# modin-project/modin

Hardware: AMD Instinct MI355X
Metric: rows/sec groupby-sum (higher is better)
Workload: dtype f64; 1 GPU; groupby-sum-1e9-int64key-f64val; rows=1000000000, key_cardinality=1000000, key_distribution=uniform, key_dtype=int64, val_dtype=float64, partitions_per_rank=1, api_layer=modin_amd.pandas DataFrame.groupby('k').sum(), parallelism=dp1

## Files before the change

include/hipframe.h:

```cpp
#ifndef HIPFRAME_H
#define HIPFRAME_H

#include <stdint.h>
#include <stddef.h>

#ifdef __cplusplus
extern "C" {
#endif

enum {
  HF_OK = 0,
  HF_ERR_HIP = 1,
  HF_ERR_ARG = 2,
  HF_ERR_NOINIT = 3,
  HF_ERR_UNSUPPORTED = 4
};

enum {
  HF_INT64 = 0,
  HF_FLOAT64 = 1
};

typedef struct hf_col hf_col;

// ... 51 lines not shown
  double  mn, mx;
  int64_t isum, imn, imx;
} hf_reduce_result;
int hf_reduce(const hf_col* in, hf_reduce_result* out);

enum { HF_AGG_SUM = 0, HF_AGG_MIN = 1, HF_AGG_MAX = 2,
       HF_AGG_PROD = 3  };
int hf_groupby_accum(const hf_col* keys,
                     const hf_col* const* vals,
                     int nvals, int agg_op,
                     int64_t key_min, int64_t n_slots,
                     uintptr_t sums, uintptr_t rowcnt, uintptr_t counts);

int hf_group_moments(const hf_col* gid,
                     const hf_col* val,
                     uintptr_t centre, int64_t n_groups, uintptr_t table);

int hf_fill_f64(uintptr_t dptr, double value, int64_t n);
int hf_fill_i64(uintptr_t dptr, int64_t value, int64_t n);

int hf_fill_randint(hf_col* col, uint64_t seed, int64_t lo, int64_t hi);
int hf_fill_randf64(hf_col* col, uint64_t seed);
int hf_fill_randcdf(hf_col* col, uint64_t seed, const hf_col* cdf);

int hf_groupby_hash_accum(const hf_col* keys, const hf_col* const* vals,
                          int nvals, int agg_op, int64_t H,
                          uintptr_t tkey, uintptr_t sums, uintptr_t rowcnt,
                          uintptr_t counts);
int hf_groupby_hash_compact(uintptr_t tkey, uintptr_t sums, uintptr_t rowcnt,
                            uintptr_t counts, int nvals, int64_t H,
                            hf_col** out_keys, hf_col** out_sums,
                            hf_col** out_counts, int64_t* n_groups);

int hf_groupby_sorted(const hf_col* sorted_keys, const hf_col* const* vals,
                      int nvals, int agg_op, int want_counts,
                      hf_col** out_keys, hf_col** out_sums,
                      hf_col** out_counts, int64_t* n_groups);

int hf_fixup_empty(const hf_col* val, const hf_col* cnt, hf_col** out);

int hf_groupby_compact(uintptr_t sums, uintptr_t rowcnt, uintptr_t counts,
                       int nvals, int64_t key_min, int64_t n_slots,
                       hf_col** out_keys,
                       hf_col** out_sums,
                       hf_col** out_counts,
                       int64_t* n_groups);

int hf_groupby_reduce(const hf_col* keys, const hf_col* const* vals,
                      int nvals, int agg_op, int want_counts,
                      int64_t key_min, int64_t n_slots,
                      hf_col** out_keys, hf_col** out_sums,
                      hf_col** out_counts, int64_t* n_groups);

typedef struct hf_join hf_join;

int hf_join_build(const hf_col* rkeys,
                  const hf_col* const* rvals,
                  int nr, int64_t key_min, int64_t n_slots, hf_join** out);
int hf_join_free(hf_join* j);

int hf_join_probe(const hf_join* j, const hf_col* lkeys,
                  hf_col** out_keys,
                  hf_col** out_lidx,
                  hf_col** out_rcols,
                  int64_t* n_out);

int hf_gather(const hf_col* col, const hf_col* idx, hf_col** out);

int hf_col_concat(const hf_col* const* cols, int ncols, hf_col** out);

int hf_col_slice(const hf_col* col, int64_t start, int64_t len, hf_col** out);

enum {
  HF_CMP_GT = 0, HF_CMP_GE = 1, HF_CMP_LT = 2, HF_CMP_LE = 3,
  HF_CMP_EQ = 4, HF_CMP_NE = 5,
  HF_CMP_NOTNA = 6
};
int hf_compare_scalar(int op, const hf_col* col, double scalar,
                      hf_col** out);

typedef struct hf_filterplan hf_filterplan;
int hf_filter_plan(const hf_col* mask, hf_filterplan** out, int64_t* n_kept);
int hf_filter_apply(const hf_filterplan* plan, const hf_col* col,
                    hf_col** out);
int hf_filter_iota(const hf_filterplan* plan, int64_t base, hf_col** out);
int hf_filter_plan_free(hf_filterplan* plan);

int hf_sort_perm(const hf_col* keys, int ascending, hf_col** out_perm);

int hf_shuffle_dest(const hf_col* keys, const int64_t* splitters, int nsplit,
                    hf_col** dest);

int hf_ordered_i64(const hf_col* col, int direction, hf_col** out);

int hf_cumsum(const hf_col* col, int agg_op, hf_col** out);

int hf_seg_cumsum(const hf_col* col, const hf_col* heads, int agg_op,
                  hf_col** out);

int hf_ewm_mean(const hf_col* col, const hf_col* heads ,
                double alpha, int adjust, int ignore_na, int64_t min_periods,
                hf_col** out);

int hf_scatter(const hf_col* col, const hf_col* idx, hf_col** out);

int hf_cross_idx(int64_t nl, int64_t nr, hf_col** lidx, hf_col** ridx);
// ... 15 lines not shown
```

modin_amd/core/lib.py:

```python

from __future__ import annotations

import ctypes as ct
import os
import threading

import numpy as np

_LIB_NAME = "libhipframe.so"


class HfError(RuntimeError):
    """Raised when a hipframe C-ABI call fails."""


class HfReduceResult(ct.Structure):
    _fields_ = [
        ("sum", ct.c_double),
        ("count", ct.c_int64),
        ("mn", ct.c_double),
        ("mx", ct.c_double),
        ("isum", ct.c_int64),
        ("imn", ct.c_int64),
        ("imx", ct.c_int64),
# ... 83 lines not shown
            "hf_groupby_hash_compact": (ct.c_int, [ct.c_size_t, ct.c_size_t,
                                                   ct.c_size_t, ct.c_size_t,
                                                   ct.c_int, ct.c_int64,
                                                   ct.POINTER(ct.c_void_p),
                                                   ct.POINTER(ct.c_void_p),
                                                   ct.POINTER(ct.c_void_p),
                                                   ct.POINTER(ct.c_int64)]),
            "hf_groupby_sorted": (ct.c_int, [ct.c_void_p,
                                             ct.POINTER(ct.c_void_p),
                                             ct.c_int, ct.c_int, ct.c_int,
                                             ct.POINTER(ct.c_void_p),
                                             ct.POINTER(ct.c_void_p),
                                             ct.POINTER(ct.c_void_p),
                                             ct.POINTER(ct.c_int64)]),
            "hf_search_sorted": (ct.c_int, [ct.c_void_p, ct.c_void_p,
                                            ct.POINTER(ct.c_void_p)]),
            "hf_ordered_i64": (ct.c_int, [ct.c_void_p, ct.c_int,
                                          ct.POINTER(ct.c_void_p)]),
            "hf_cumsum": (ct.c_int, [ct.c_void_p, ct.c_int,
                                     ct.POINTER(ct.c_void_p)]),
            "hf_seg_cumsum": (ct.c_int, [ct.c_void_p, ct.c_void_p, ct.c_int,
                                         ct.POINTER(ct.c_void_p)]),
            "hf_ewm_mean": (ct.c_int, [ct.c_void_p, ct.c_void_p, ct.c_double,
                                       ct.c_int, ct.c_int, ct.c_int64,
                                       ct.POINTER(ct.c_void_p)]),
            "hf_scatter": (ct.c_int, [ct.c_void_p, ct.c_void_p,
                                      ct.POINTER(ct.c_void_p)]),
            "hf_cross_idx": (ct.c_int, [ct.c_int64, ct.c_int64,
                                        ct.POINTER(ct.c_void_p),
                                        ct.POINTER(ct.c_void_p)]),
            "hf_shuffle_dest": (ct.c_int, [ct.c_void_p,
                                           ct.POINTER(ct.c_int64), ct.c_int,
                                           ct.POINTER(ct.c_void_p)]),
            "hf_memcpy_dd": (ct.c_int, [ct.c_size_t, ct.c_size_t,
                                        ct.c_int64]),
            "hf_sort_perm": (ct.c_int, [ct.c_void_p, ct.c_int,
                                        ct.POINTER(ct.c_void_p)]),
            "hf_fixup_empty": (ct.c_int, [ct.c_void_p, ct.c_void_p,
                                          ct.POINTER(ct.c_void_p)]),
            "hf_groupby_compact": (ct.c_int, [ct.c_size_t, ct.c_size_t, ct.c_size_t,
                                              ct.c_int, ct.c_int64, ct.c_int64,
                                              ct.POINTER(ct.c_void_p),
                                              ct.POINTER(ct.c_void_p),
                                              ct.POINTER(ct.c_void_p),
                                              ct.POINTER(ct.c_int64)]),
            "hf_groupby_reduce": (ct.c_int, [ct.c_void_p,
                                             ct.POINTER(ct.c_void_p),
                                             ct.c_int, ct.c_int, ct.c_int,
                                             ct.c_int64, ct.c_int64,
                                             ct.POINTER(ct.c_void_p),
                                             ct.POINTER(ct.c_void_p),
                                             ct.POINTER(ct.c_void_p),
                                             ct.POINTER(ct.c_int64)]),
            "hf_col_concat": (ct.c_int, [ct.POINTER(ct.c_void_p), ct.c_int,
                                         ct.POINTER(ct.c_void_p)]),
            "hf_col_slice": (ct.c_int, [ct.c_void_p, ct.c_int64, ct.c_int64,
                                        ct.POINTER(ct.c_void_p)]),
            "hf_join_build": (ct.c_int, [ct.c_void_p, ct.POINTER(ct.c_void_p),
                                         ct.c_int, ct.c_int64, ct.c_int64,
                                         ct.POINTER(ct.c_void_p)]),
            "hf_join_free": (ct.c_int, [ct.c_void_p]),
            "hf_join_probe": (ct.c_int, [ct.c_void_p, ct.c_void_p,
                                         ct.POINTER(ct.c_void_p),
                                         ct.POINTER(ct.c_void_p),
                                         ct.POINTER(ct.c_void_p),
                                         ct.POINTER(ct.c_int64)]),
            "hf_gather": (ct.c_int, [ct.c_void_p, ct.c_void_p,
                                     ct.POINTER(ct.c_void_p)]),
            "hf_compare_scalar": (ct.c_int, [ct.c_int, ct.c_void_p,
                                             ct.c_double,
                                             ct.POINTER(ct.c_void_p)]),
            "hf_filter_plan": (ct.c_int, [ct.c_void_p, ct.POINTER(ct.c_void_p),
                                          ct.POINTER(ct.c_int64)]),
            "hf_filter_apply": (ct.c_int, [ct.c_void_p, ct.c_void_p,
                                           ct.POINTER(ct.c_void_p)]),
            "hf_filter_iota": (ct.c_int, [ct.c_void_p, ct.c_int64,
                                          ct.POINTER(ct.c_void_p)]),
            "hf_filter_plan_free": (ct.c_int, [ct.c_void_p]),
            "hf_profiling": (ct.c_int, [ct.c_int]),
            "hf_kernel_stats": (ct.c_int, [ct.c_char_p, ct.POINTER(ct.c_int64),
                                           ct.POINTER(ct.c_double)]),
            "hf_kernel_stats_reset": (ct.c_int, []),
        }
        for name, (res, args) in sig.items():
            fn = getattr(dll, name)
            fn.restype = res
            fn.argtypes = args
        _dll = dll
        return dll


def exported_symbols():
    return [
        "hf_init", "hf_shutdown", "hf_device_count", "hf_last_error", "hf_sync",
        "hf_put", "hf_get", "hf_col_alloc", "hf_col_free", "hf_col_len",
        "hf_col_dtype", "hf_col_dptr", "hf_alloc_raw", "hf_free_raw",
        "hf_memset_raw", "hf_dev_live", "hf_map_scalar", "hf_map_scalar_i64",
        "hf_binary",
        "hf_reduce", "hf_groupby_accum", "hf_group_moments",
        "hf_groupby_compact", "hf_groupby_reduce", "hf_fill_f64",
        "hf_fixup_empty", "hf_sort_perm", "hf_fill_i64",
        "hf_fill_randint", "hf_fill_randf64", "hf_fill_randcdf",
        "hf_groupby_hash_accum", "hf_groupby_hash_compact",
        "hf_groupby_sorted", "hf_shuffle_dest", "hf_memcpy_dd",
        "hf_search_sorted", "hf_ordered_i64", "hf_cumsum", "hf_seg_cumsum",
        "hf_ewm_mean", "hf_scatter", "hf_cross_idx",
        "hf_col_concat", "hf_col_slice", "hf_join_build", "hf_join_free", "hf_join_probe",
        "hf_gather", "hf_compare_scalar", "hf_filter_plan", "hf_filter_apply",
        "hf_filter_iota", "hf_filter_plan_free", "hf_profiling",
        "hf_kernel_stats", "hf_kernel_stats_reset",
    ]


def _check(rc: int, what: str) -> None:
    if rc != 0:
        msg = load().hf_last_error().decode() if _dll else "?"
        raise HfError(f"{what} failed (rc={rc}): {msg}")


def ensure_ready(gpu: int | None = None) -> None:
    global _inited_gpu
    dll = load()
    if gpu is None:
        gpu = int(os.environ.get("MODIN_AMD_GPU", "0"))
    with _lock:
        if _inited_gpu == gpu:
            return
        _check(dll.hf_init(gpu), "hf_init")
        _inited_gpu = gpu


def is_ready() -> bool:
    return _inited_gpu is not None


def shutdown() -> None:
    global _inited_gpu
    if _dll is not None and _inited_gpu is not None:
        _dll.hf_shutdown()
    _inited_gpu = None


def device_count() -> int:
    dll = load()
    n = ct.c_int(0)
    dll.hf_device_count(ct.byref(n))
    return n.value


class ColumnRef:

    __slots__ = ("handle", "length", "dtype_code", "_reduce_cache")

# ... 260 lines not shown
    ensure_ready()
    out = ct.c_void_p()
    _check(load().hf_fixup_empty(val.handle, cnt.handle, ct.byref(out)),
           "hf_fixup_empty")
    return _wrap(out, val.length, HF_FLOAT64)


def groupby_compact(sums: int, rowcnt: int, counts: int, nvals: int,
                    key_min: int, n_slots: int):
    ensure_ready()
    out_keys = ct.c_void_p()
    out_sums = (ct.c_void_p * max(nvals, 1))()
    out_counts = (ct.c_void_p * max(nvals, 1))()
    n_groups = ct.c_int64(0)
    _check(load().hf_groupby_compact(sums, rowcnt, counts, nvals, key_min,
                                     n_slots, ct.byref(out_keys), out_sums,
                                     out_counts if counts else None,
                                     ct.byref(n_groups)), "hf_groupby_compact")
    n = n_groups.value
    kcol = _wrap(out_keys, n, HF_INT64)
    scols = [_wrap(ct.c_void_p(out_sums[c]), n, HF_FLOAT64) for c in range(nvals)]
    ccols = ([_wrap(ct.c_void_p(out_counts[c]), n, HF_INT64) for c in range(nvals)]
             if counts else None)
    return kcol, scols, ccols, n


def is_native_col(col) -> bool:
    return (_dll is not None and _inited_gpu is not None
            and isinstance(col, ColumnRef))


def groupby_reduce(keys: ColumnRef, vals: list, agg_op: int,
                   want_counts: bool, key_min: int, n_slots: int):
    ensure_ready()
    nvals = len(vals)
    arr = (ct.c_void_p * max(nvals, 1))(*[v.handle for v in vals])
    out_keys = ct.c_void_p()
    out_sums = (ct.c_void_p * max(nvals, 1))()
    out_counts = (ct.c_void_p * max(nvals, 1))()
    n_groups = ct.c_int64(0)
    _check(load().hf_groupby_reduce(keys.handle, arr, nvals, agg_op,
                                    1 if want_counts else 0, key_min, n_slots,
                                    ct.byref(out_keys), out_sums,
                                    out_counts if want_counts else None,
                                    ct.byref(n_groups)), "hf_groupby_reduce")
    n = n_groups.value
    kcol = _wrap(out_keys, n, HF_INT64)
    scols = [_wrap(ct.c_void_p(out_sums[c]), n, HF_FLOAT64) for c in range(nvals)]
    ccols = ([_wrap(ct.c_void_p(out_counts[c]), n, HF_INT64)
              for c in range(nvals)] if want_counts else None)
    return kcol, scols, ccols, n


def col_slice(col: ColumnRef, start: int, length: int) -> ColumnRef:
    ensure_ready()
    out = ct.c_void_p()
    _check(load().hf_col_slice(col.handle, start, length, ct.byref(out)),
           "hf_col_slice")
    return _wrap(out, length, col.dtype_code)


def concat(cols: list) -> ColumnRef:
    ensure_ready()
    arr = (ct.c_void_p * len(cols))(*[c.handle for c in cols])
    out = ct.c_void_p()
    _check(load().hf_col_concat(arr, len(cols), ct.byref(out)), "hf_col_concat")
    return _wrap(out, sum(c.length for c in cols), cols[0].dtype_code)


class JoinRef:

    __slots__ = ("handle", "nr", "rdtypes")

    def __init__(self, handle, nr, rdtypes):
        self.handle = handle
        self.nr = nr
        self.rdtypes = rdtypes

    def __del__(self):
        try:
            if _dll is not None and _inited_gpu is not None and self.handle:
                _dll.hf_join_free(self.handle)
        except Exception:
            pass


def join_build(rkeys: ColumnRef, rvals: list, key_min: int,
               n_slots: int) -> JoinRef:
    ensure_ready()
    arr = (ct.c_void_p * max(len(rvals), 1))(*[v.handle for v in rvals])
    out = ct.c_void_p()
    _check(load().hf_join_build(rkeys.handle, arr, len(rvals), key_min,
                                n_slots, ct.byref(out)), "hf_join_build")
    return JoinRef(out, len(rvals), [v.dtype_code for v in rvals])


def join_probe(j: JoinRef, lkeys: ColumnRef):
    ensure_ready()
    out_keys = ct.c_void_p()
    out_lidx = ct.c_void_p()
    out_r = (ct.c_void_p * max(j.nr, 1))()
    n_out = ct.c_int64(0)
    _check(load().hf_join_probe(j.handle, lkeys.handle, ct.byref(out_keys),
                                ct.byref(out_lidx), out_r, ct.byref(n_out)),
           "hf_join_probe")
    n = n_out.value
# ... 178 lines not shown
```

modin_amd/csrc/hipframe.hip:

```cpp

#include <hip/hip_runtime.h>
#include <algorithm>
#include <cstdint>
#include <cstdio>
#include <cstring>
#include <cstdlib>
#include <memory>
#include <string>
#include <type_traits>
#include <unordered_map>
#include <utility>
#include <vector>

#include "../../include/hipframe.h"


struct GbKeyCache {
  std::vector<int64_t> hist;
  int64_t hist_kmin = 0;
  int64_t hist_nb = 0;
  int64_t hist_nslots = 0;
  void*   d_k32 = nullptr;
  int64_t k32_min = 0;
  void*   d_curinit = nullptr;
// ... 86 lines not shown
    float ms = 0.f;
    hipEventElapsedTime(&ms, p.a, p.b);
    auto& s = g.stats[p.name];
    s.first += 1;
    s.second += ms;
    hipEventDestroy(p.a);
    hipEventDestroy(p.b);
  }
  g.pending.clear();
  return HF_OK;
}

template <typename F>
int timed_launch(const char* name, F&& launch) {
  if (!g.profiling) {
    launch();
    hipError_t e = hipGetLastError();
    if (e != hipSuccess) return set_hip_err(name, e);
    return HF_OK;
  }
  TimedPair p;
  p.name = name;
  HF_HIP(name, hipEventCreate(&p.a));
  HF_HIP(name, hipEventCreate(&p.b));
  HF_HIP(name, hipEventRecord(p.a, g.stream));
  launch();
  hipError_t e = hipGetLastError();
  if (e != hipSuccess) return set_hip_err(name, e);
  HF_HIP(name, hipEventRecord(p.b, g.stream));
  g.pending.push_back(p);
  if (g.pending.size() > 4096) return resolve_stats(name);
  return HF_OK;
}

template <int V>
using int_tag = std::integral_constant<int, V>;
template <typename F>
int with_bool(bool b, F&& f) {
  return b ? f(std::true_type{}) : f(std::false_type{});
}
template <typename F>
int with_aop(int agg_op, F&& f) {
  return agg_op == HF_AGG_SUM   ? f(int_tag<HF_AGG_SUM>{})
         : agg_op == HF_AGG_MIN ? f(int_tag<HF_AGG_MIN>{})
                                : f(int_tag<HF_AGG_MAX>{});
}
template <int MAX, int N = 0, typename F>
int with_nvals(int nv, F&& f) {
  if (nv == N) return f(int_tag<N>{});
  if constexpr (N < MAX)
    return with_nvals<MAX, N + 1>(nv, std::forward<F>(f));
  else
    return set_err(HF_ERR_ARG, "with_nvals", "column count out of range");
}
template <typename F>
int with_scan_op(int agg_op, F&& f) {
  return agg_op == HF_AGG_PROD ? f(int_tag<HF_AGG_PROD>{})
                               : with_aop(agg_op, std::forward<F>(f));
}
template <typename F>
int with_dtype(int dtype, F&& f) {
  return dtype == HF_FLOAT64 ? f(double{}) : f(int64_t{});
}

constexpr int BLOCK = 256;
constexpr int64_t GRID_CAP = 4096;

int64_t grid_for(int64_t work_items) {
  int64_t b = (work_items + BLOCK - 1) / BLOCK;
  if (b < 1) b = 1;
  return b < GRID_CAP ? b : GRID_CAP;
}

}


namespace {
inline bool sync_alloc() {
  static int v = -1;
  if (v < 0) v = getenv("HF_SYNC_ALLOC") ? 1 : 0;
  return v == 1;
}

struct DevCache {
  std::unordered_map<int64_t, std::vector<void*>> free_by_size;
  std::unordered_map<void*, int64_t> size_of;
  int64_t cached_bytes = 0;

  hipError_t alloc(void** p, int64_t bytes) {
    bytes = (bytes + 255) & ~255LL;
    auto it = free_by_size.find(bytes);
    if (it != free_by_size.end() && !it->second.empty()) {
      *p = it->second.back();
      it->second.pop_back();
      cached_bytes -= bytes;
      return hipSuccess;
    }
    hipError_t e = hipMalloc(p, bytes);
    if (e == hipErrorOutOfMemory) {
      trim();
      e = hipMalloc(p, bytes);
    }
    if (e == hipSuccess) size_of[*p] = bytes;
    return e;
  }
  void free(void* p) {
// ... 761 lines not shown
    for (int j = 0; j < TABR; ++j) {
      const int t = j * BLK + threadIdx.x;
      if (t < tabw) traw[j] = row[t];
    }
  };

  int64_t tile = blockIdx.x;
  if (tile < ntiles) issue_loads(tile);
  for (; tile < ntiles; tile += gridDim.x) {
    __syncthreads();
#pragma unroll
    for (int j = 0; j < PAIRS; ++j) {
      const int64_t pj = tile * (TILE / 2) + (int64_t)j * BLK + threadIdx.x;
      if (pj < npair_total) {
        const unsigned pa = draw[j] & 0xFFFFu, pb = draw[j] >> 16;
        if (pa < (unsigned)TILE) sval[pa] = vraw[j].x;
        if (pb < (unsigned)TILE) sval[pb] = vraw[j].y;
      }
    }
#pragma unroll
    for (int j = 0; j < TABR; ++j) {
      const int t = j * BLK + threadIdx.x;
      if (t < tabw) it_off[t] = traw[j];
    }
    __syncthreads();
    const int64_t nxt = tile + gridDim.x;
    if (nxt < ntiles) issue_loads(nxt);
    const int staged = (int)it_off[nb];
    int b[RPT];
#pragma unroll
    for (int j = 0; j < RPT; ++j) b[j] = 0;
    for (int s = search0; s > 0; s >>= 1) {
#pragma unroll
      for (int j = 0; j < RPT; ++j) {
        const int p = j * BLK + threadIdx.x;
        const int m = b[j] + s;
        if (p < staged && m < nb && it_off[m] <= (unsigned)p) b[j] = m;
      }
    }
#pragma unroll
    for (int j = 0; j < RPT; ++j) {
      const int p = j * BLK + threadIdx.x;
      if (p < staged)
        r0[(int64_t)it_gbase[b[j]] + ((unsigned)p - it_off[b[j]])] = sval[p];
    }
  }
}

__global__ void k_gb_plan_err(const unsigned long long* __restrict__ meta,
                              unsigned long long* __restrict__ err) {
  if (blockIdx.x == 0 && threadIdx.x == 0 && meta[1]) atomicAdd(err, meta[1]);
}

template <bool ROWCNT, bool CNT, bool HAVE_VAL, int RL, int AOP,
          bool PART = false>
__global__ void __launch_bounds__(512) k_gb_bucket_agg(
    const double* __restrict__ vals, const unsigned short* __restrict__ lowkeys,
    const GbWorkItem* __restrict__ work, int64_t n_slots,
    double* __restrict__ gsums, unsigned long long* __restrict__ growcnt,
    unsigned long long* __restrict__ gcounts,
    double* __restrict__ part_sums = nullptr,
    unsigned* __restrict__ part_cnt = nullptr) {
  static_assert(!PART || (HAVE_VAL && !ROWCNT), "PART flushes value tables");
  constexpr int RANGE = 1 << RL;
  __shared__ __attribute__((aligned(16))) double lsums[HAVE_VAL ? RANGE : 1];
  __shared__ __attribute__((aligned(16))) unsigned lcnt[CNT ? RANGE : 1];
  __shared__ unsigned char ltouch[PART ? 1 : RANGE];
  const GbWorkItem w = work[blockIdx.x];
  for (int s = threadIdx.x; s < RANGE; s += blockDim.x) {
    if (HAVE_VAL) lsums[s] = agg_identity<AOP>();
    if (!PART) ltouch[s] = 0;
    if (CNT) lcnt[s] = 0;
  }
  __syncthreads();
  const int64_t end = w.start + w.len;
  auto one_row = [&](int64_t i) {
    const int slot = lowkeys[i];
    if (!PART) ltouch[slot] = 1;
    if (HAVE_VAL) {
      const double v = vals[i];
      if (v == v) {
        lds_slot_agg<AOP>(&lsums[slot], v);
        if (CNT) atomicAdd(&lcnt[slot], 1u);
      }
    }
  };
  const int64_t a0 = w.start;
  const int64_t npair = (end - a0) >> 1;
  const ushort2* k2 = reinterpret_cast<const ushort2*>(lowkeys + a0);
  const double2* v2 = reinterpret_cast<const double2*>(vals + a0);
  int rslot = -1;
  double racc = 0.0;
  unsigned rcnt = 0;
  auto flush = [&]() {
    if (rslot >= 0) {
      lds_slot_agg<AOP>(&lsums[rslot], racc);
      if (CNT) atomicAdd(&lcnt[rslot], rcnt);
    }
    rslot = -1;
    rcnt = 0;
  };
  auto feed = [&](int slot, double v) {
    if (!PART) ltouch[slot] = 1;
    if (HAVE_VAL && v == v) {
      if (slot == rslot) {
        racc = AOP == HF_AGG_SUM ? racc + v
               : AOP == HF_AGG_MIN ? fmin(racc, v) : fmax(racc, v);
        ++rcnt;
      } else {
        flush();
        rslot = slot;
        racc = v;
        rcnt = 1;
      }
    }
  };
// ... 2316 lines not shown
        constexpr int BLK = NV < 2 ? GB_PLAN_BLK : 512;
        constexpr int64_t TILE = (int64_t)BLK * GB_PLAN_RPT;
        const uint32_t sgrid = gb_tile_grid(((n & ~1LL) + TILE - 1) / TILE);
        const uint32_t lds =
            (uint32_t)(TILE * (8 * NV + 4) + a.nb * 12 + 16);
        return timed_launch(REC ? "gb_plan_record" : "gb_scatter", [&] {
          hipLaunchKernelGGL(
              (k_gb_scatter<NV, GB_PLAN_RPT, BLK, RL, REC>), dim3(sgrid),
              dim3(BLK), lds, g.stream, (const int64_t*)a.keys->dptr,
              (const unsigned*)kc.d_k32, ptrs.vals[0], ptrs.vals[1], n,
              a.key_min, a.n_slots, (int)a.nb, a.d_cur, a.r0, a.r1, a.rk,
              a.d_err, rec);
        });
      });
  if (REC && rc == HF_OK) {
    kc.plan_kmin = a.key_min;
    kc.plan_nslots = a.n_slots;
    kc.plan_rl = RL;
  }
  return rc;
}

int radix_replay(const GbRadixCall& a, const double* v, bool add_err) {
  const GbKeyCache& kc = a.keys->gb;
  const int64_t n = a.keys->len;
  int search0 = 0;
  for (int s = 1; s <= a.nb - 1; s <<= 1) search0 = s;
  const uint32_t lds =
      (uint32_t)((int64_t)GB_PLAN_TILE * 8 + (2 * a.nb + 1) * 4);
  return timed_launch("gb_scatter", [&] {
    hipLaunchKernelGGL((k_gb_replay<GB_PLAN_RPT, GB_PLAN_BLK>),
                       dim3(gb_tile_grid(gb_plan_tiles(n))), dim3(GB_PLAN_BLK),
                       lds, g.stream, (const unsigned short*)kc.d_plan_dst, v,
                       n, (int)a.nb, search0, (const unsigned*)kc.d_plan_tab,
                       (const unsigned long long*)kc.d_plan_meta, a.r0,
                       a.d_err, add_err ? 1 : 0);
  });
}

int radix_plan_err(const GbRadixCall& a) {
  return timed_launch("gb_plan_err", [&] {
    hipLaunchKernelGGL(k_gb_plan_err, dim3(1), dim3(64), 0, g.stream,
                       (const unsigned long long*)a.keys->gb.d_plan_meta,
                       a.d_err);
  });
}

template <int RL, int AOP, bool R, bool C, bool V>
int radix_agg(const GbRadixCall& a, const double* v, double* gs,
              unsigned long long* growcnt, unsigned long long* gc) {
  const GbKeyCache& kc = a.keys->gb;
  return timed_launch("gb_bucket_agg", [&] {
    hipLaunchKernelGGL((k_gb_bucket_agg<R, C, V, RL, AOP>),
                       dim3((uint32_t)kc.work_n), dim3(512), 0, g.stream, v,
                       a.rk, (const GbWorkItem*)kc.d_work, a.n_slots, gs,
                       growcnt, gc);
  });
}

int gb_radix_rl(int64_t n_slots, bool want_cnt) {
  const int64_t nb13 = (n_slots + (1 << 13) - 1) >> 13;
  const int64_t nb12 = (n_slots + (1 << 12) - 1) >> 12;
  return (!want_cnt && nb13 <= GB_MAX_BUCKETS) ? 13
         : (want_cnt && nb12 <= GB_MAX_BUCKETS) ? 12
         : (nb13 <= GB_MAX_BUCKETS) ? 13 : 0;
}

template <int RL, int AOP>
int gb_radix_mapped(hf_col* keys, const GbPtrs& ptrs, int nvals,
                    int64_t key_min, int64_t n_slots, bool want_counts,
                    GroupOut& o) {
  const GbKeyCache& kc = keys->gb;
  const int64_t ng = kc.n_groups;
  int rc = o.keys.alloc(ng, HF_INT64);
  if (rc != HF_OK) return rc;
  if (ng > 0)
    HF_HIP("hf_groupby_reduce",
           hipMemcpyAsync(o.keys.data<void>(), kc.d_gkeys, ng * 8,
                          hipMemcpyDeviceToDevice, g.stream));
  if (nvals == 0) return HF_OK;
  constexpr int64_t RANGE = 1 << RL;
  const int64_t nb = (n_slots + RANGE - 1) >> RL;
  DevBuf r0, part_sums, part_cnt;
  HF_HIP("hf_groupby_reduce", r0.alloc(radix_alloc_rows(kc) * 8));
  HF_HIP("hf_groupby_reduce", part_sums.alloc(kc.work_n * RANGE * 8));
  if (want_counts)
    HF_HIP("hf_groupby_reduce", part_cnt.alloc(kc.work_n * RANGE * 4));
  const GbRadixCall a{keys, nb, key_min, n_slots, nullptr, r0.as<double>(),
                      nullptr, (unsigned short*)kc.d_plan_rk, nullptr};
  for (int c = 0; c < nvals; ++c) {
    rc = o.sums[c].alloc(ng, HF_FLOAT64);
    if (rc == HF_OK && want_counts) rc = o.cnts[c].alloc(ng, HF_INT64);
    if (rc == HF_OK) rc = radix_replay(a, ptrs.vals[c], false);
    if (rc != HF_OK) return rc;
    rc = with_bool(want_counts, [&](auto cTag) {
      constexpr bool C = decltype(cTag)::value;
      int r = timed_launch("gb_bucket_agg", [&] {
        hipLaunchKernelGGL(
            (k_gb_bucket_agg<false, C, true, RL, AOP, true>),
            dim3((uint32_t)kc.work_n), dim3(512), 0, g.stream, a.r0, a.rk,
            (const GbWorkItem*)kc.d_work, n_slots, nullptr, nullptr, nullptr,
            part_sums.as<double>(), part_cnt.as<unsigned>());
      });
      if (r != HF_OK) return r;
      return timed_launch("gb_compact_scatter", [&] {
        hipLaunchKernelGGL(
            (k_gb_combine<RL, AOP, C>),
            dim3((uint32_t)((n_slots + BLOCK - 1) / BLOCK)), dim3(BLOCK), 0,
            g.stream, (const unsigned*)kc.d_gidx, (const unsigned*)kc.d_item0,
            part_sums.as<double>(), part_cnt.as<unsigned>(), n_slots,
            o.sums[c].data<double>(),
            C ? o.cnts[c].data<int64_t>() : nullptr);
      });
    });
    if (rc != HF_OK) return rc;
  }
  return HF_OK;
}

template <int RL, int AOP>
int gb_radix_path(hf_col* keys, const GbPtrs& ptrs, int nvals, int64_t key_min,
                  int64_t n_slots, uintptr_t sums, uintptr_t rowcnt,
                  uintptr_t counts, unsigned long long* d_err,
                  bool with_rowcnt = true) {
  GbKeyCache& kc = keys->gb;
  const int64_t nb = (n_slots + (1 << RL) - 1) >> RL;
  int rc = ensure_host_hist(keys, key_min, n_slots, nb, RL);
  if (rc != HF_OK) return rc;
  rc = ensure_radix_layout<RL>(keys, nb);
  if (rc != HF_OK) return rc;
  const GbPlan mode = ensure_plan(keys, RL, key_min, n_slots, nb);
  if (mode == GbPlan::None) {
    rc = ensure_keys32(keys, key_min);
    if (rc != HF_OK) return rc;
  }
  const int64_t rows = radix_alloc_rows(kc);
  DevBuf r0, r1, rk, d_cur;
  if (nvals > 0) HF_HIP("gb_radix", r0.alloc(rows * 8));
  if (mode == GbPlan::None) {
    if (nvals > 1) HF_HIP("gb_radix", r1.alloc(rows * 8));
    HF_HIP("gb_radix", rk.alloc(rows * 2));
  }
  if (mode != GbPlan::Replay) {
    HF_HIP("gb_radix", d_cur.alloc(nb * 4));
    HF_HIP("gb_radix", hipMemcpyAsync(d_cur.as<void>(), kc.d_curinit, nb * 4,
                                      hipMemcpyDeviceToDevice, g.stream));
  }
  const GbRadixCall a{keys, nb, key_min, n_slots, d_err, r0.as<double>(),
                      r1.as<double>(),
                      mode == GbPlan::None ? rk.as<unsigned short>()
                                           : (unsigned short*)kc.d_plan_rk,
                      d_cur.as<unsigned>()};
  if (mode == GbPlan::None)
    rc = radix_scatter<RL, false>(a, ptrs, nvals);
  else if (mode == GbPlan::Record)
    rc = radix_scatter<RL, true>(a, ptrs, nvals);
  else if (nvals == 0 || kc.work_n == 0)
    rc = radix_plan_err(a);
  if (rc != HF_OK || kc.work_n == 0) return rc;
  unsigned long long* growcnt = (unsigned long long*)rowcnt;
  if (nvals == 0)
    return radix_agg<RL, AOP, true, false, false>(a, nullptr, nullptr, growcnt,
                                                  nullptr);
  const bool cnt = counts != 0;
  for (int c = 0; c < nvals; ++c) {
    if (mode == GbPlan::Replay || (mode == GbPlan::Record && c > 0)) {
      rc = radix_replay(a, ptrs.vals[c], mode == GbPlan::Replay && c == 0);
      if (rc != HF_OK) return rc;
    }
    const double* v = (c == 0 || mode != GbPlan::None) ? a.r0 : a.r1;
    double* gs = (double*)sums + (int64_t)c * n_slots;
    unsigned long long* gc =
        cnt ? (unsigned long long*)counts + (int64_t)c * n_slots : nullptr;
    rc = with_bool(c == 0 && with_rowcnt, [&](auto rTag) {
      return with_bool(cnt, [&](auto cTag) {
        return radix_agg<RL, AOP, decltype(rTag)::value,
                         decltype(cTag)::value, true>(a, v, gs, growcnt, gc);
      });
    });
    if (rc != HF_OK) return rc;
  }
  return HF_OK;
}

}

extern "C" {

int hf_groupby_accum(const hf_col* keys, const hf_col* const* vals, int nvals,
                     int agg_op, int64_t key_min, int64_t n_slots,
                     uintptr_t sums, uintptr_t rowcnt, uintptr_t counts) {
  HF_NEED_INIT("hf_groupby_accum");
  if (!keys || !vals || nvals < 0 || nvals > GB_MAX_VALS)
    return set_err(HF_ERR_ARG, "hf_groupby_accum", "bad args (nvals<=8)");
  if (agg_op < HF_AGG_SUM || agg_op > HF_AGG_MAX)
    return set_err(HF_ERR_ARG, "hf_groupby_accum", "bad agg_op");
  if (keys->dtype != HF_INT64)
    return set_err(HF_ERR_ARG, "hf_groupby_accum", "keys must be int64");
  if (n_slots <= 0) return set_err(HF_ERR_ARG, "hf_groupby_accum", "n_slots<=0");
  GbPtrs ptrs{};
  for (int c = 0; c < nvals; ++c) {
    if (!vals[c] || vals[c]->dtype != HF_FLOAT64 || vals[c]->len != keys->len)
      return set_err(HF_ERR_ARG, "hf_groupby_accum",
                     "vals must be float64 columns of keys' length");
    ptrs.vals[c] = (const double*)vals[c]->dptr;
  }
  const int64_t n = keys->len;
  unsigned long long* d_err = scratch_at(SCRATCH_GB_ERR);
  auto route = [&](auto aopTag) -> int {
    constexpr int AOP = decltype(aopTag)::value;
    if (n > 0 && n_slots <= GB_DENSE_MAX)
      return gb_dense_path<AOP>(keys, ptrs, nvals, key_min, n_slots, sums,
                                rowcnt, counts, d_err);
    const int rl_ok = gb_radix_rl(n_slots, counts != 0);
    if (n > 0 && rl_ok) {
      int rc2 = HF_OK;
      for (int c0 = 0; c0 < (nvals ? nvals : 1) && rc2 == HF_OK; c0 += 2) {
        GbPtrs sub{};
        const int nv = nvals == 0 ? 0 : std::min(2, nvals - c0);
        for (int c = 0; c < nv; ++c) sub.vals[c] = ptrs.vals[c0 + c];
        const uintptr_t ssub = sums + (uintptr_t)c0 * n_slots * 8;
        const uintptr_t csub =
            counts ? counts + (uintptr_t)c0 * n_slots * 8 : 0;
        auto radix = [&](auto rlTag) {
          return gb_radix_path<decltype(rlTag)::value ? 13 : 12, AOP>(
              const_cast<hf_col*>(keys), sub, nv, key_min, n_slots, ssub,
              rowcnt, csub, d_err, c0 == 0);
        };
        rc2 = with_bool(rl_ok == 13, radix);
        if (nvals == 0) break;
      }
      return rc2;
    }
    return -1;
  };
  int routed = with_aop(agg_op, route);
  if (routed != -1) return routed;
  return with_nvals<GB_MAX_VALS>(nvals, [&](auto nvTag) {
    return with_bool(counts != 0, [&](auto cntTag) {
      return with_aop(agg_op, [&](auto aopTag) {
        return timed_launch("gb_accum", [&] {
          hipLaunchKernelGGL((k_gb_accum<decltype(nvTag)::value,
                                         decltype(cntTag)::value,
                                         decltype(aopTag)::value>),
                             dim3(grid_for((n >> 1) + 1)), dim3(BLOCK), 0,
                             g.stream, (const int64_t*)keys->dptr, ptrs, n,
                             key_min, n_slots, (double*)sums,
                             (unsigned long long*)rowcnt,
                             (unsigned long long*)counts, d_err);
        });
      });
    });
  });
}

int hf_group_moments(const hf_col* gid, const hf_col* val, uintptr_t centre,
                     int64_t n_groups, uintptr_t table) {
  HF_NEED_INIT("hf_group_moments");
  if (!val || val->dtype != HF_FLOAT64 || !centre || !table)
    return set_err(HF_ERR_ARG, "hf_group_moments",
                   "val must be float64; centre/table must be non-null");
  if (n_groups <= 0)
    return set_err(HF_ERR_ARG, "hf_group_moments", "n_groups<=0");
  if (gid && (gid->dtype != HF_INT64 || gid->len != val->len))
    return set_err(HF_ERR_ARG, "hf_group_moments",
                   "gid must be an int64 column of val's length");
  if (!gid && n_groups != 1)
    return set_err(HF_ERR_ARG, "hf_group_moments",
                   "a null gid means one group (n_groups must be 1)");
  const int64_t n = val->len;
  if (n == 0) return HF_OK;
  const double* d_val = (const double*)val->dptr;
  const double* d_c = (const double*)centre;
  double* d_tab = (double*)table;
  if (!gid) {
    int64_t grid = grid_for((n >> 1) + 1);
    if (grid > 1024) grid = 1024;
    return timed_launch("gm_one", [&] {
      hipLaunchKernelGGL(k_gm_one, dim3((uint32_t)grid), dim3(BLOCK), 0,
                         g.stream, d_val, n, d_c, d_tab);
    });
  }
// ... 78 lines not shown
    h_sum_ptrs[c] = o.sums[c].data<double>();
    if (want_counts) {
      rc = o.cnts[c].alloc(total, HF_INT64);
      if (rc != HF_OK) return rc;
      h_cnt_ptrs[c] = o.cnts[c].data<int64_t>();
    }
  }
  DevBuf sum_ptrs_buf, cnt_ptrs_buf;
  HF_HIP("hf_groupby_compact",
         sum_ptrs_buf.alloc(sizeof(double*) * (nvals ? nvals : 1)));
  HF_HIP("hf_groupby_compact",
         cnt_ptrs_buf.alloc(sizeof(int64_t*) * (nvals ? nvals : 1)));
  double** d_sum_ptrs = sum_ptrs_buf.as<double*>();
  int64_t** d_cnt_ptrs = cnt_ptrs_buf.as<int64_t*>();
  HF_HIP("hf_groupby_compact",
         hipMemcpyAsync(d_sum_ptrs, h_sum_ptrs.data(), sizeof(double*) * nvals,
                        hipMemcpyHostToDevice, g.stream));
  if (want_counts)
    HF_HIP("hf_groupby_compact",
           hipMemcpyAsync(d_cnt_ptrs, h_cnt_ptrs.data(), sizeof(int64_t*) * nvals,
                          hipMemcpyHostToDevice, g.stream));
  rc = with_bool(want_counts, [&](auto cTag) {
    return timed_launch("gb_compact_scatter", [&] {
      hipLaunchKernelGGL(k_compact_scatter<decltype(cTag)::value>,
                         dim3((uint32_t)ntiles), dim3(BLOCK), 0, g.stream,
                         (const double*)sums, (const unsigned long long*)rowcnt,
                         (const unsigned long long*)counts, nvals, key_min,
                         n_slots, d_tiles, o.keys.data<int64_t>(), d_sum_ptrs,
                         d_cnt_ptrs);
    });
  });
  if (rc != HF_OK) return rc;
  if (gidx) {
    rc = timed_launch("gb_gidx", [&] {
      hipLaunchKernelGGL(k_gb_gidx, dim3((uint32_t)ntiles), dim3(BLOCK), 0,
                         g.stream, (const unsigned long long*)rowcnt, n_slots,
                         d_tiles, gidx);
    });
    if (rc != HF_OK) return rc;
  }
  o.commit(out_keys, out_sums, out_counts);
  *n_groups = total;
  return HF_OK;
}

int hf_groupby_compact(uintptr_t sums, uintptr_t rowcnt, uintptr_t counts,
                       int nvals, int64_t key_min, int64_t n_slots,
                       hf_col** out_keys, hf_col** out_sums, hf_col** out_counts,
                       int64_t* n_groups) {
  return gb_compact(sums, rowcnt, counts, nvals, key_min, n_slots, out_keys,
                    out_sums, out_counts, n_groups, nullptr);
}

int hf_groupby_reduce(const hf_col* keys, const hf_col* const* vals, int nvals,
                      int agg_op, int want_counts, int64_t key_min,
                      int64_t n_slots, hf_col** out_keys, hf_col** out_sums,
                      hf_col** out_counts, int64_t* n_groups) {
  HF_NEED_INIT("hf_groupby_reduce");
  if (!keys || !vals || nvals < 0 || nvals > GB_MAX_VALS || !out_keys ||
      !n_groups || (nvals > 0 && !out_sums) || (want_counts && !out_counts))
    return set_err(HF_ERR_ARG, "hf_groupby_reduce", "bad args (nvals<=8)");
  if (agg_op < HF_AGG_SUM || agg_op > HF_AGG_MAX)
    return set_err(HF_ERR_ARG, "hf_groupby_reduce", "bad agg_op");
  if (keys->dtype != HF_INT64)
    return set_err(HF_ERR_ARG, "hf_groupby_reduce", "keys must be int64");
  if (n_slots <= 0)
    return set_err(HF_ERR_ARG, "hf_groupby_reduce", "n_slots<=0");
  GbPtrs ptrs{};
  for (int c = 0; c < nvals; ++c) {
    if (!vals[c] || vals[c]->dtype != HF_FLOAT64 || vals[c]->len != keys->len)
      return set_err(HF_ERR_ARG, "hf_groupby_reduce",
                     "vals must be float64 columns of keys' length");
    ptrs.vals[c] = (const double*)vals[c]->dptr;
  }
  hf_col* kcol = const_cast<hf_col*>(keys);
  GbKeyCache& kc = kcol->gb;
  const bool cnt = want_counts != 0;
  const int rl = (keys->len > 0 && n_slots > GB_DENSE_MAX)
                     ? gb_radix_rl(n_slots, cnt) : 0;
  const bool plan_ok = rl != 0 && kc.plan_rl == rl &&
                       kc.plan_kmin == key_min && kc.plan_nslots == n_slots;
  if (plan_ok && kc.d_gidx) {
    GroupOut o(nvals, cnt);
    const int rc = with_aop(agg_op, [&](auto aopTag) {
      return with_bool(rl == 13, [&](auto rlTag) {
        return gb_radix_mapped<decltype(rlTag)::value ? 13 : 12,
                               decltype(aopTag)::value>(
            kcol, ptrs, nvals, key_min, n_slots, cnt, o);
      });
    });
    if (rc != HF_OK) return rc;
    o.commit(out_keys, out_sums, out_counts);
    *n_groups = kc.n_groups;
    return HF_OK;
  }
  const int64_t tab = (int64_t)(nvals ? nvals : 1) * n_slots;
  DevBuf sums, rowcnt, counts, gidx;
  HF_HIP("hf_groupby_reduce", sums.alloc(tab * 8));
  HF_HIP("hf_groupby_reduce", rowcnt.alloc(n_slots * 8));
  if (cnt) HF_HIP("hf_groupby_reduce", counts.alloc(tab * 8));
  int rc = HF_OK;
  if (agg_op == HF_AGG_SUM)
    HF_HIP("hf_groupby_reduce",
           hipMemsetAsync(sums.as<void>(), 0, tab * 8, g.stream));
  else
    rc = hf_fill_f64((uintptr_t)sums.as<void>(),
                     agg_op == HF_AGG_MIN ? INFINITY : -INFINITY, tab);
  if (rc != HF_OK) return rc;
  HF_HIP("hf_groupby_reduce",
         hipMemsetAsync(rowcnt.as<void>(), 0, n_slots * 8, g.stream));
  if (cnt)
    HF_HIP("hf_groupby_reduce",
           hipMemsetAsync(counts.as<void>(), 0, tab * 8, g.stream));
  rc = hf_groupby_accum(keys, vals, nvals, agg_op, key_min, n_slots,
                        (uintptr_t)sums.as<void>(),
                        (uintptr_t)rowcnt.as<void>(),
                        (uintptr_t)counts.as<void>());
  if (rc != HF_OK) return rc;
  const bool arm = rl != 0 && kc.plan_rl == rl && kc.plan_kmin == key_min &&
                   kc.plan_nslots == n_slots && kc.work_n > 0 && !kc.d_gidx;
  if (arm && gidx.alloc(n_slots * 4) != hipSuccess) (void)hipGetLastError();
  hf_col* okeys = nullptr;
  rc = gb_compact((uintptr_t)sums.as<void>(), (uintptr_t)rowcnt.as<void>(),
                  (uintptr_t)counts.as<void>(), nvals, key_min, n_slots,
                  &okeys, out_sums, out_counts, n_groups, gidx.as<unsigned>());
  if (rc != HF_OK) return rc;
  *out_keys = okeys;
  if (gidx.as<void>() && *n_groups > 0) {
    DevBuf gkeys;
    if (gkeys.alloc(*n_groups * 8) != hipSuccess) {
      (void)hipGetLastError();
    } else if (hipMemcpyAsync(gkeys.as<void>(), okeys->dptr, *n_groups * 8,
                              hipMemcpyDeviceToDevice, g.stream) ==
               hipSuccess) {
      kc.d_gidx = gidx.release();
      kc.d_gkeys = gkeys.release();
      kc.n_groups = *n_groups;
    }
  }
// ... 1167 lines not shown
```

Measured before the change: 173.9 billion rows/s.

## Add 16384-slot radix buckets with 1024-thread blocks for large key ranges

Introduces a radix level of 14 bits (16384 slots per bucket held in LDS) for count-free groupby when the key range exceeds 2^18, and launches the bucket-aggregation kernel with 1024 threads at that level. Larger buckets mean fewer buckets and work items, so there are fewer partition passes and less per-bucket overhead. The cost is a 128KB LDS sums table per block, which can lower occupancy, and count-carrying aggregations cannot use this level. An environment variable can force the old 13-bit level, and a C entry point exposes the chosen level to Python.

```diff
diff --git a/include/hipframe.h b/include/hipframe.h
--- a/include/hipframe.h
+++ b/include/hipframe.h
@@ -127,6 +127,8 @@
                       hf_col** out_keys, hf_col** out_sums,
                       hf_col** out_counts, int64_t* n_groups);
 
+int hf_groupby_radix_rl(int64_t n_slots, int want_counts);
+
 typedef struct hf_join hf_join;
 
 int hf_join_build(const hf_col* rkeys,
diff --git a/modin_amd/core/lib.py b/modin_amd/core/lib.py
--- a/modin_amd/core/lib.py
+++ b/modin_amd/core/lib.py
@@ -159,6 +159,7 @@
                                              ct.POINTER(ct.c_void_p),
                                              ct.POINTER(ct.c_void_p),
                                              ct.POINTER(ct.c_int64)]),
+            "hf_groupby_radix_rl": (ct.c_int, [ct.c_int64, ct.c_int]),
             "hf_col_concat": (ct.c_int, [ct.POINTER(ct.c_void_p), ct.c_int,
                                          ct.POINTER(ct.c_void_p)]),
             "hf_col_slice": (ct.c_int, [ct.c_void_p, ct.c_int64, ct.c_int64,
@@ -205,7 +206,8 @@
         "hf_memset_raw", "hf_dev_live", "hf_map_scalar", "hf_map_scalar_i64",
         "hf_binary",
         "hf_reduce", "hf_groupby_accum", "hf_group_moments",
-        "hf_groupby_compact", "hf_groupby_reduce", "hf_fill_f64",
+        "hf_groupby_compact", "hf_groupby_reduce", "hf_groupby_radix_rl",
+        "hf_fill_f64",
         "hf_fixup_empty", "hf_sort_perm", "hf_fill_i64",
         "hf_fill_randint", "hf_fill_randf64", "hf_fill_randcdf",
         "hf_groupby_hash_accum", "hf_groupby_hash_compact",
@@ -572,6 +574,10 @@
     return kcol, scols, ccols, n
 
 
+def groupby_radix_rl(n_slots: int, want_counts: bool) -> int:
+    return load().hf_groupby_radix_rl(n_slots, 1 if want_counts else 0)
+
+
 def col_slice(col: ColumnRef, start: int, length: int) -> ColumnRef:
     ensure_ready()
     out = ct.c_void_p()
diff --git a/modin_amd/csrc/hipframe.hip b/modin_amd/csrc/hipframe.hip
--- a/modin_amd/csrc/hipframe.hip
+++ b/modin_amd/csrc/hipframe.hip
@@ -162,6 +162,11 @@
     return with_nvals<MAX, N + 1>(nv, std::forward<F>(f));
   else
     return set_err(HF_ERR_ARG, "with_nvals", "column count out of range");
+}
+template <typename F>
+int with_rl(int rl, F&& f) {
+  return rl == 14 ? f(int_tag<14>{})
+         : rl == 13 ? f(int_tag<13>{}) : f(int_tag<12>{});
 }
 template <typename F>
 int with_scan_op(int agg_op, F&& f) {
@@ -1029,9 +1034,11 @@
   if (blockIdx.x == 0 && threadIdx.x == 0 && meta[1]) atomicAdd(err, meta[1]);
 }
 
+constexpr int gb_p2_block(int rl) { return rl >= 14 ? 1024 : 512; }
+
 template <bool ROWCNT, bool CNT, bool HAVE_VAL, int RL, int AOP,
           bool PART = false>
-__global__ void __launch_bounds__(512) k_gb_bucket_agg(
+__global__ void __launch_bounds__(gb_p2_block(RL)) k_gb_bucket_agg(
     const double* __restrict__ vals, const unsigned short* __restrict__ lowkeys,
     const GbWorkItem* __restrict__ work, int64_t n_slots,
     double* __restrict__ gsums, unsigned long long* __restrict__ growcnt,
@@ -1039,6 +1046,8 @@
     double* __restrict__ part_sums = nullptr,
     unsigned* __restrict__ part_cnt = nullptr) {
   static_assert(!PART || (HAVE_VAL && !ROWCNT), "PART flushes value tables");
+  static_assert(RL <= 16, "low keys are u16");
+  static_assert(RL <= 13 || !CNT, "no LDS for a counts table beside 16384 sums");
   constexpr int RANGE = 1 << RL;
   __shared__ __attribute__((aligned(16))) double lsums[HAVE_VAL ? RANGE : 1];
   __shared__ __attribute__((aligned(16))) unsigned lcnt[CNT ? RANGE : 1];
@@ -3461,18 +3470,37 @@
   const GbKeyCache& kc = a.keys->gb;
   return timed_launch("gb_bucket_agg", [&] {
     hipLaunchKernelGGL((k_gb_bucket_agg<R, C, V, RL, AOP>),
-                       dim3((uint32_t)kc.work_n), dim3(512), 0, g.stream, v,
+                       dim3((uint32_t)kc.work_n), dim3(gb_p2_block(RL)), 0,
+                       g.stream, v,
                        a.rk, (const GbWorkItem*)kc.d_work, a.n_slots, gs,
                        growcnt, gc);
   });
 }
 
+constexpr int64_t GB_RL14_ABOVE = 1 << 18;
 int gb_radix_rl(int64_t n_slots, bool want_cnt) {
+  static const bool rl14_env = [] {
+    const char* e = getenv("HF_GB_RL");
+    return !(e && strcmp(e, "13") == 0);
+  }();
   const int64_t nb13 = (n_slots + (1 << 13) - 1) >> 13;
   const int64_t nb12 = (n_slots + (1 << 12) - 1) >> 12;
-  return (!want_cnt && nb13 <= GB_MAX_BUCKETS) ? 13
-         : (want_cnt && nb12 <= GB_MAX_BUCKETS) ? 12
+  if (!want_cnt && nb13 <= GB_MAX_BUCKETS)
+    return (rl14_env && n_slots > GB_RL14_ABOVE) ? 14 : 13;
+  return (want_cnt && nb12 <= GB_MAX_BUCKETS) ? 12
          : (nb13 <= GB_MAX_BUCKETS) ? 13 : 0;
+}
+
+template <int RL, typename F>
+int with_cnt(bool cnt, F&& f) {
+  if constexpr (RL >= 14) {
+    if (cnt)
+      return set_err(HF_ERR_UNSUPPORTED, "gb_radix",
+                     "16384-slot buckets carry no counts");
+    return f(std::false_type{});
+  } else {
+    return with_bool(cnt, std::forward<F>(f));
+  }
 }
 
 template <int RL, int AOP>
@@ -3502,13 +3530,14 @@
     if (rc == HF_OK && want_counts) rc = o.cnts[c].alloc(ng, HF_INT64);
     if (rc == HF_OK) rc = radix_replay(a, ptrs.vals[c], false);
     if (rc != HF_OK) return rc;
-    rc = with_bool(want_counts, [&](auto cTag) {
+    rc = with_cnt<RL>(want_counts, [&](auto cTag) {
       constexpr bool C = decltype(cTag)::value;
       int r = timed_launch("gb_bucket_agg", [&] {
         hipLaunchKernelGGL(
             (k_gb_bucket_agg<false, C, true, RL, AOP, true>),
-            dim3((uint32_t)kc.work_n), dim3(512), 0, g.stream, a.r0, a.rk,
-            (const GbWorkItem*)kc.d_work, n_slots, nullptr, nullptr, nullptr,
+            dim3((uint32_t)kc.work_n), dim3(gb_p2_block(RL)), 0, g.stream,
+            a.r0, a.rk, (const GbWorkItem*)kc.d_work, n_slots, nullptr,
+            nullptr, nullptr,
             part_sums.as<double>(), part_cnt.as<unsigned>());
       });
       if (r != HF_OK) return r;
@@ -3582,7 +3611,7 @@
     unsigned long long* gc =
         cnt ? (unsigned long long*)counts + (int64_t)c * n_slots : nullptr;
     rc = with_bool(c == 0 && with_rowcnt, [&](auto rTag) {
-      return with_bool(cnt, [&](auto cTag) {
+      return with_cnt<RL>(cnt, [&](auto cTag) {
         return radix_agg<RL, AOP, decltype(rTag)::value,
                          decltype(cTag)::value, true>(a, v, gs, growcnt, gc);
       });
@@ -3632,11 +3661,11 @@
         const uintptr_t csub =
             counts ? counts + (uintptr_t)c0 * n_slots * 8 : 0;
         auto radix = [&](auto rlTag) {
-          return gb_radix_path<decltype(rlTag)::value ? 13 : 12, AOP>(
+          return gb_radix_path<decltype(rlTag)::value, AOP>(
               const_cast<hf_col*>(keys), sub, nv, key_min, n_slots, ssub,
               rowcnt, csub, d_err, c0 == 0);
         };
-        rc2 = with_bool(rl_ok == 13, radix);
+        rc2 = with_rl(rl_ok, radix);
         if (nvals == 0) break;
       }
       return rc2;
@@ -3821,6 +3850,10 @@
                     out_sums, out_counts, n_groups, nullptr);
 }
 
+int hf_groupby_radix_rl(int64_t n_slots, int want_counts) {
+  return n_slots > 0 ? gb_radix_rl(n_slots, want_counts != 0) : 0;
+}
+
 int hf_groupby_reduce(const hf_col* keys, const hf_col* const* vals, int nvals,
                       int agg_op, int want_counts, int64_t key_min,
                       int64_t n_slots, hf_col** out_keys, hf_col** out_sums,
@@ -3852,8 +3885,8 @@
   if (plan_ok && kc.d_gidx) {
     GroupOut o(nvals, cnt);
     const int rc = with_aop(agg_op, [&](auto aopTag) {
-      return with_bool(rl == 13, [&](auto rlTag) {
-        return gb_radix_mapped<decltype(rlTag)::value ? 13 : 12,
+      return with_rl(rl, [&](auto rlTag) {
+        return gb_radix_mapped<decltype(rlTag)::value,
                                decltype(aopTag)::value>(
             kcol, ptrs, nvals, key_min, n_slots, cnt, o);
       });
```

Result: faster. 180.2 billion rows/s (median of 6 runs) (+3.6%).
